# nannau/DoWnGAN

Measured on AMD Instinct MI355X. Metric: train-step samples/sec (G+D+GP), higher is better.
Workload: dtype bf16

## Files before the change

downgan_amd/_lib.py:

```python
from __future__ import annotations

import ctypes as C
import os

_HERE = os.path.dirname(os.path.abspath(__file__))
LIB_PATH = os.environ.get("DG_LIB_OVERRIDE") or os.path.join(_HERE, "csrc", "libdowngan_hip.so")

DG_F32, DG_BF16 = 0, 1
STATUS = {0: "DG_OK", -1: "DG_ERR_BAD_SHAPE", -2: "DG_ERR_BAD_DTYPE", -3: "DG_ERR_BAD_ARG", -4: "DG_ERR_LAUNCH"}


class Epilogue(C.Structure):
    _fields_ = [("bias", C.c_void_p), ("has_act", C.c_int), ("act_slope", C.c_float),
                ("r1", C.c_void_p), ("ldr1", C.c_int64), ("s1", C.c_float),
                ("r2", C.c_void_p), ("ldr2", C.c_int64), ("s2", C.c_float),
                ("mask", C.c_void_p), ("ldmask", C.c_int64), ("mask_slope", C.c_float),
                ("accumulate", C.c_int), ("mask_bits", C.c_void_p), ("out_bits", C.c_void_p),
                ("mask_c0", C.c_int), ("mask_last", C.c_int), ("out_q", C.c_void_p), ("out_qs", C.c_void_p), ("ldqs", C.c_int64),
                ("out_u", C.c_void_p), ("out_ue", C.c_void_p), ("skip_y", C.c_int), ("out_amax", C.c_void_p)]


class ConvGeom(C.Structure):
    _fields_ = [("dtype", C.c_int), ("N", C.c_int), ("H", C.c_int), ("W", C.c_int),
                ("Cin", C.c_int), ("Cout", C.c_int), ("stride", C.c_int), ("cin_real", C.c_int), ("pixel_shuffle", C.c_int),
# ... 48 lines not shown
EOF_MAX_C, EOF_MAX_K = 8, 64
RAPSD_MAX_N = 2048


class EofFields(C.Structure):
    _fields_ = [("base", C.c_void_p), ("dtype", C.c_int), ("T", C.c_int), ("C", C.c_int), ("P", C.c_int),
                ("ld_t", C.c_int64), ("ld_c", C.c_int64), ("ld_p", C.c_int64)]


MINMAX_PARTS = 256
_vp, _i, _i64, _f = C.c_void_p, C.c_int, C.c_int64, C.c_float
_PROTOS = {
    "dg_conv3x3_fwd": [C.POINTER(ConvGeom), C.POINTER(Epilogue), _vp, _vp, _vp, _vp],
    "dg_conv3x3_dgrad": [C.POINTER(ConvGeom), C.POINTER(Epilogue), _vp, _vp, _vp, _vp],
    "dg_conv3x3_wgrad": [C.POINTER(ConvGeom), _vp, _vp, _vp, _vp, _vp],
    "dg_conv3x3_wgrad_dense": [_vp, _i, _vp, _vp, _vp, _vp, _vp],
    "dg_conv3x3_wgrad_f8": [C.POINTER(ConvGeom), _vp, _vp, _vp, _vp, _vp, _vp],
    "dg_exp_from_amax": [_vp, _i, _i, _vp, _vp],
    "dg_conv3x3_wgrad_dense_f8": [C.POINTER(ConvGeom), _i, _vp, _vp, _vp, _vp, _vp, _vp],
    "dg_gather_gemm": [C.POINTER(GGDesc), C.POINTER(Epilogue), _vp, _vp, _vp, _vp],
    "dg_conv3x3_plan": [C.POINTER(ConvGeom), _i, C.POINTER(GGDesc)],
    "dg_last_conv_kernels": [],
    "dg_conv3x3_dgrad_launches": [C.POINTER(ConvGeom)],
    "dg_colsum": [_i, _vp, _i64, _i64, _i64, _i64, _i, _vp, _vp],
    "dg_colsum_multi": [_i, _vp, _i64, _i64, _i, _i, _vp, _vp],
    "dg_repack_conv_weights": [_i, _i, _vp, _vp, _i, _i, _vp],
    "dg_repack_dense_dgrad": [_i, _vp, _i, _i, _vp, _vp],
    "dg_wgrad_unswap": [_vp, _vp, _i, _i, _vp],
    "dg_linear_fwd": [_i, _vp, _i64, _vp, _i64, _vp, _i, _i, _i, _i64, _vp],
    "dg_linear_dx": [_i, _i, _vp, _i, _vp, _i64, _vp, _i64, _vp, _i64, _f, _i, _i, _i64, _vp],
    "dg_linear_dw": [_i, _vp, _i, _vp, _i64, _vp, _i64, _i, _i, _i64, _vp],
    "dg_linear_dw_wide": [_i, _vp, _i, _vp, _i64, _vp, _i64, _i, _i, _i64, _i, _vp],
    "dg_bias_act": [_i, _vp, _i, _vp, _vp, _i, _i, _i, _i, _f, _vp, _i, _f, _vp],
    "dg_mask_mul": [_i, _vp, _i64, _vp, _i64, _i64, _i, _f, _vp],
    "dg_axpby": [_i, _vp, _i64, _vp, _i64, _f, _vp, _i64, _f, _i64, _i, _vp],
    "dg_gp_interp": [_i, _vp, _vp, _vp, _vp, _i, _i64, _vp],
    "dg_gp_interp_c2": [_i, _vp, _vp, _i64, _vp, _vp, _vp, _vp, _i, _i64, _vp],
    "dg_scale_rows_c2": [_i, _vp, _i64, _vp, _vp, _i, _i64, _vp],
    "dg_sumsq_rows": [_i, _vp, _i, _i64, _vp, _vp],
    "dg_gp_finish": [_vp, _i, _i, _f, _f, _vp, _vp, _vp],
    "dg_scale_rows": [_i, _vp, _vp, _vp, _i, _i64, _vp],
    "dg_l1": [_i, _vp, _i64, _vp, _i64, _i64, _i, _vp, _vp, _i64, _f, _vp, _i64, _vp],
    "dg_sqdiff": [_i, _vp, _i64, _vp, _i64, _i64, _i, _vp, _vp],
    "dg_sum_strided": [_vp, _i, _i, _f, _vp, _vp],
    "dg_fill_col": [_vp, _i, _i, _i, _f, _vp],
    "dg_adam": [_vp, _vp, _vp, _vp, _vp, _i64, _f, _f, _f, _f, _i, _f, _vp],
# ... 94 lines not shown
```

downgan_amd/csrc/conv_halo.hip:

```cpp
#include "gg_common.h"

#ifdef DG_STAMP
__device__ unsigned long long g_stamps[2 * 8 * 12];
extern "C" int dg_debug_stamps(unsigned long long* out) {
  return hipMemcpyFromSymbol(out, HIP_SYMBOL(g_stamps), sizeof(g_stamps)) == hipSuccess ? 0 : 1;
}
#define DG_WGLOG_MAX 16384
__device__ unsigned long long g_wglog[DG_WGLOG_MAX * 3];
extern "C" int dg_debug_wglog(unsigned long long* out, int n) {
  return hipMemcpyFromSymbol(out, HIP_SYMBOL(g_wglog), sizeof(unsigned long long) * 3 * (n < DG_WGLOG_MAX ? n : DG_WGLOG_MAX)) == hipSuccess ? 0 : 1;
}
#define STAMP(v) do { __builtin_amdgcn_sched_barrier(0); v = __builtin_amdgcn_s_memtime(); __builtin_amdgcn_sched_barrier(0); } while (0)
#else
#define STAMP(v) do { } while (0)
#endif
bool gg_regroup_taps_by_plane(GGArgs& a) {
  if (a.ntaps != 9) return false;
  unsigned codes[9], out[9];
  bool seen[3][3] = {};
  for (int t = 0; t < 9; ++t) {
    codes[t] = t < 8 ? (unsigned)((a.tap_lo >> (8 * t)) & 0xffull) : (a.tap_hi & 0xffu);
    const int dy = (int)(codes[t] & 3u) - 1, dx = (int)((codes[t] >> 2) & 3u) - 1;
    if (dy < -1 || dy > 1 || dx < -1 || dx > 1 || seen[dy + 1][dx + 1]) return false;
    seen[dy + 1][dx + 1] = true;
  }
  int n = 0;
  for (int plane = 0; plane < 4; ++plane)
    for (int t = 0; t < 9; ++t) {
      const int dy = (int)(codes[t] & 3u) - 1, dx = (int)((codes[t] >> 2) & 3u) - 1;
      if ((dy != 0) * 2 + (dx != 0) != plane) continue;
      const unsigned by = dy == -1 ? 0u : 1u, bx = dx == -1 ? 0u : 1u;
      out[n++] = by | (bx << 2) | (codes[t] & 0xf0u);
    }
  a.tap_lo = 0; a.tap_hi = 0;
  for (int t = 0; t < 9; ++t) {
    if (t < 8) a.tap_lo |= (unsigned long long)out[t] << (8 * t); else a.tap_hi = out[t];
  }
  return true;
}

template <typename T, bool S2, bool PS = false, int NW = 4, bool SEG = false>
__global__ __launch_bounds__(64 * NW, 2) void gg_halo4w_kernel(const GGArgs a, int tiles_x, int tiles_y) {
  static_assert(!SEG || (!S2 && !PS && NW == 4), "SEG is a mode of the plain four-wave kernel");
  constexpr int NT = 64 * NW, RPP = NT / 8;
  constexpr int EPC = DT<T>::EPC;
  constexpr int ES = (int)sizeof(T);
  constexpr int TH = 16, TW = 16, PW = TW + 2, PROWS = (TH + 2) * PW;
  constexpr int BC = 32 * NW, KC = 8;
  constexpr int PITCH = KC * 16 + 16;
  constexpr int WROW = KC * 16;
  constexpr int NPL = (PROWS * KC + NT - 1) / NT;
  constexpr int NWL = BC * KC / NT;
  extern __shared__ __attribute__((aligned(16))) char dsm4w[];
  char* const s_patch = dsm4w;
  char* const s_w = dsm4w + PROWS * PITCH;

  const int tid = threadIdx.x, lane = tid & 63, wave = __builtin_amdgcn_readfirstlane(tid >> 6);
  const unsigned tile = SEG ? blockIdx.x : xcd_remap(blockIdx.x, a.nwg);
  const int tile_c = tile % a.nct;
  unsigned rest = tile / a.nct;
  const int tx0 = (rest % tiles_x) * TW; rest /= tiles_x;
  int cls = 0;
  if (SEG && a.seg == 2) { cls = (int)(rest & 3u); rest >>= 2; }
  const int ty0 = (rest % tiles_y) * TH; rest /= tiles_y;
  if (SEG && a.seg != 2) { cls = (int)(rest & 3u); rest >>= 2; }
  const int img = (int)rest;
  const int ntaps_l = SEG ? (0x4221 >> (4 * cls)) & 15 : a.ntaps;
  const int tap0_l = SEG ? (0x5310 >> (4 * cls)) & 15 : 0;
  const int c0 = tile_c * BC;
  const int cc = tid & 7, r0 = tid >> 3;
  const int wq = wave & 3, wh = wave >> 2;
  const int sy_base = S2 ? (ty0 > 0 ? 2 * (ty0 - 1) : 0) : (ty0 - 1 > 0 ? ty0 - 1 : 0);
  const char* Xb = PS ? reinterpret_cast<const char*>(a.x) + ((long long)img * 2 * a.Hs + 2 * sy_base) * (2 * a.Ws) * a.ldx * ES
                      : reinterpret_cast<const char*>(a.x) + ((long long)img * a.Hs + sy_base) * a.Ws * a.ldx * ES;
  const char* Wb = reinterpret_cast<const char*>(a.w) + (long long)c0 * a.ldw * ES;
  const int l15 = lane & 15, g = lane >> 4;
  const int ncbr = a.cch / KC;
  const int ncb = S2 ? 4 * ncbr : ncbr;
  const int nsteps = ncbr * ntaps_l;
  auto plane_of = [&](int vcb) { return S2 ? (int)(vcb >= ncbr) + (int)(vcb >= 2 * ncbr) + (int)(vcb >= 3 * ncbr) : 0; };
  auto ntaps_of = [&](int vcb) { return S2 ? (0x4221 >> (4 * plane_of(vcb))) & 15 : ntaps_l; };

  unsigned woff[NWL];
#pragma unroll
  for (int i = 0; i < NWL; ++i) {
    int row = wave * 32 + i * 8 + (lane >> 3);
    const int logical = (lane & 7) ^ ((row >> 1) & 7);
    row = perm64(row);
    if (c0 + row >= a.Nout) row = a.Nout - 1 - c0;
    woff[i] = (unsigned)((long long)row * a.ldw * ES) + logical * 16;
  }
  auto tap_code = [&](int vcb, int tap) {
    const int gt = S2 ? ((0x5310 >> (4 * plane_of(vcb))) & 15) + tap : tap0_l + tap;
    return gt < 8 ? (unsigned)((a.tap_lo >> (8 * gt)) & 0xffull) : (a.tap_hi & 0xffu);
  };
  constexpr int K1 = RPP / PW, K2 = RPP % PW;
  const int p_rstep = (S2 ? 2 : PS ? 4 : 1) * a.Ws * a.ldx * ES, p_cstep = ((S2 || PS) ? 2 : 1) * a.ldx * ES;
  const int p_A = K1 * p_rstep + K2 * p_cstep, p_Bd = p_rstep - PW * p_cstep;
  unsigned p_off0, p_wlo = 0, p_whb = 0;
  {
    const int py0 = r0 / PW, px0 = r0 - py0 * PW;
    const int o_rows = S2 ? 2 * (ty0 - 1) - sy_base : PS ? 4 * (ty0 - 1 - sy_base) : ty0 - 1 - sy_base;
    const int o_cols = (S2 || PS) ? 2 * (tx0 - 1) : tx0 - 1;
    p_off0 = (unsigned)((o_rows * a.Ws + o_cols) * a.ldx * ES + py0 * p_rstep + px0 * p_cstep) + cc * 16;
    const unsigned hlim = S2 ? (unsigned)a.Hs >> 1 : (unsigned)a.Hs, wlim = S2 ? (unsigned)a.Ws >> 1 : (unsigned)a.Ws;
#pragma unroll
    for (int i = 0; i < NPL; ++i) {
      const int w = (px0 + i * K2) / PW;
      const int py = py0 + i * K1 + w, px = px0 + i * K2 - w * PW;
      const bool ok = r0 + RPP * i < PROWS && (unsigned)(ty0 - 1 + py) < hlim && (unsigned)(tx0 - 1 + px) < wlim;
      if (i < 8) p_wlo |= (unsigned)w << (4 * i); else p_whb |= (unsigned)w << (4 * (i - 8));
      if (!ok) p_whb |= 1u << (16 + i);
    }
  }
  asm volatile("" : "+v"(p_off0), "+v"(p_wlo), "+v"(p_whb));
  u32x4_t rp[NPL];
  auto load_patch = [&](int vcb) {
    const int plane = plane_of(vcb), cb = vcb - plane * ncbr;
    const int ppy = plane >> 1, ppx = plane & 1;
    const int psq = PS ? (cb * KC) / a.cps_src_chunks : 0;
    const int psy = psq >> 1, psx = psq & 1;
    long long cboff = PS ? (long long)(cb * KC - psq * a.cps_src_chunks) * EPC * ES : (long long)cb * KC * EPC * ES;
    if (S2) cboff += (long long)(ppy * a.Ws + ppx) * a.ldx * ES;
    if (PS) cboff += (long long)(psy * 2 * a.Ws + psx) * a.ldx * ES;
    const unsigned long long xbase = (unsigned long long)(Xb + cboff);
    const unsigned long long xuni = ((unsigned long long)(unsigned)__builtin_amdgcn_readfirstlane((int)(unsigned)(xbase >> 32)) << 32) |
                                    (unsigned)__builtin_amdgcn_readfirstlane((int)(unsigned)xbase);
    __amdgpu_buffer_rsrc_t rx = __builtin_amdgcn_make_buffer_rsrc((void*)xuni, 0, (int)DG_OOB_OFF, 0x00020000);
#pragma unroll
    for (int i = 0; i < NPL; ++i) {
      const int w = (int)__builtin_amdgcn_ubfe(i < 8 ? p_wlo : p_whb, i < 8 ? 4 * i : 4 * (i - 8), 4);
      const unsigned bad = (unsigned)__builtin_amdgcn_sbfe((int)p_whb, 16 + i, 1);
      const unsigned off = ((unsigned)__mul24(w, p_Bd) + p_off0 + (unsigned)(i * p_A)) | bad;
      rp[i] = __builtin_amdgcn_raw_buffer_load_b128(rx, off, 0, 0);
      __builtin_amdgcn_sched_barrier(0);
    }
  };
  char* const st_base = s_patch + r0 * PITCH + cc * 16;
  auto store_patch = [&]() {
#pragma unroll
    for (int i = 0; i < NPL; ++i) {
      const int pr = r0 + RPP * i;
      if (pr < PROWS) *reinterpret_cast<uint4*>(st_base + i * RPP * PITCH) = __builtin_bit_cast(uint4, rp[i]);
    }
  };
  typedef int i32x4h_t __attribute__((ext_vector_type(4)));
  i32x4h_t w_rs;
  int w_dst0 = 0;
  auto dma_setup = [&](int vcb, int tap, int slot) {
    const unsigned code = tap_code(vcb, tap);
    const long long wo = (long long)(code >> 4) * a.Cred + (vcb - plane_of(vcb) * ncbr) * KC * EPC;
    const unsigned long long wbase = (unsigned long long)(Wb + wo * ES);
    w_rs[0] = __builtin_amdgcn_readfirstlane((int)(unsigned)wbase);
    w_rs[1] = __builtin_amdgcn_readfirstlane((int)(unsigned)(wbase >> 32) & 0xffff);
    w_rs[2] = (int)DG_OOB_OFF;
    w_rs[3] = 0x00020000;
    w_dst0 = __builtin_amdgcn_readfirstlane(
        (int)(unsigned long long)((__attribute__((address_space(3))) char*)(s_w + slot * (BC * WROW) + (wave * 32) * WROW)));
  };
  auto dma_piece = [&](int i) {
    asm volatile("s_mov_b32 m0, %0\n\ts_nop 0\n\tbuffer_load_dwordx4 %1, %2, 0 offen lds"
                 :: "s"(w_dst0 + i * 8 * WROW), "v"(woff[i]), "s"(w_rs) : "memory");
  };
  auto dma_w = [&](int cb, int tap, int slot) {
    dma_setup(cb, tap, slot);
#pragma unroll
    for (int i = 0; i < NWL; ++i) dma_piece(i);
  };
  auto barrier_all = [&]() { asm volatile("s_waitcnt vmcnt(0)" ::: "memory"); __syncthreads(); };
  auto barrier_keep_patch = [&]() { asm volatile("s_waitcnt vmcnt(%0)" :: "n"(NPL) : "memory"); __syncthreads(); };

  constexpr bool PREB = sizeof(T) == 2;
  f32x4_t acc[8][4];
#pragma unroll
  for (int j = 0; j < 8; ++j) {
    f32x4_t b = f32x4_t{0.f, 0.f, 0.f, 0.f};
    const int cbq = c0 + (tid >> 8) * 128 + (j >> 2) * 64 + 16 * ((tid & 63) >> 4) + 4 * (j & 3);
    if (PREB && a.bias && cbq < a.Nout) { const float4 b4 = *reinterpret_cast<const float4*>(a.bias + cbq); b = f32x4_t{b4.x, b4.y, b4.z, b4.w}; }
#pragma unroll
    for (int i = 0; i < 4; ++i) acc[j][i] = b;
  }

  const char* fa_k[2];
#pragma unroll
  for (int kk = 0; kk < 2; ++kk) fa_k[kk] = s_w + (wh * 128 + l15) * WROW + (((kk * 4 + g) ^ ((l15 >> 1) & 7)) * 16);
  const char* const fb_lane = s_patch + l15 * PITCH + g * 16;
  auto read_frags = [&](uint4 (&fa)[8], uint4 (&fb)[4], int pa, const char* pb, int kk) {
#pragma unroll
    for (int j = 0; j < 8; ++j) fa[j] = *reinterpret_cast<const uint4*>(fa_k[kk] + pa + j * 16 * WROW);
#pragma unroll
    for (int i = 0; i < 4; ++i) fb[i] = *reinterpret_cast<const uint4*>(pb + i * PW * PITCH + kk * 64);
  };
  auto mma_rows = [&](const uint4 (&fa)[8], const uint4 (&fb)[4], int j0) {
#pragma unroll
    for (int j = j0; j < j0 + 2; ++j)
#pragma unroll
      for (int i = 0; i < 4; ++i) Mma<T>::run(fa[j], fb[i], acc[j][i]);
  };
  auto adv = [&](int& c_, int& t_) { if (++t_ == ntaps_of(c_)) { t_ = 0; ++c_; } };
  auto patch_ptr = [&](int vcb_, int tap_) -> const char* {
    const unsigned code = tap_code(vcb_, tap_);
    const int dy = (int)(code & 3u) - 1, dx = (int)((code >> 2) & 3u) - 1;
    return fb_lane + ((wq * 4 + 1 + dy) * PW + 1 + dx) * PITCH;
  };
// ... 1 lines not shown
#ifdef DG_STAMP
  unsigned long long tK0 = 0, tA = 0, tB = 0, tC = 0, tD = 0, tE = 0, sAB = 0, sBC = 0, sCD = 0, sDE = 0, tL0 = 0;
  STAMP(tK0);
#endif
  load_patch(0);
  int cb = 0, tap = 0, cbw = 0, tapw = 0;
  dma_w(0, 0, 0);
  adv(cbw, tapw);
  if (nsteps > 1) dma_w(cbw, tapw, 1);
  adv(cbw, tapw);
  store_patch();
  barrier_all();
  uint4 fa[8], fb[4];
  const char* pb = patch_ptr(0, 0);
  int pa = 0;
  read_frags(fa, fb, pa, pb, 0);
  STAMP(tL0);
  for (int s = 0; s < nsteps; ++s) {
    STAMP(tA);
    const bool more = s + 1 < nsteps;
    int ntap = tap + 1, ncbn = cb;
    const int ntaps_cb = ntaps_of(cb);
    if (ntap == ntaps_cb) { ntap = 0; ncbn = cb + 1; }
    const bool swap = ntap == 0 && more;
    const bool patch_now = cb + 1 < ncb && (ntaps_cb == 1 || tap == 0);
    const bool fetch = s + 2 < nsteps;
#pragma unroll
    for (int q = 0; q < 4; ++q) {
      mma_rows(fa, fb, 2 * q);
      asm volatile("" : "+v"(acc[2 * q][0]), "+v"(acc[2 * q][1]), "+v"(acc[2 * q][2]), "+v"(acc[2 * q][3]),
                        "+v"(acc[2 * q + 1][0]), "+v"(acc[2 * q + 1][1]), "+v"(acc[2 * q + 1][2]), "+v"(acc[2 * q + 1][3]) :: "memory");
      __builtin_amdgcn_sched_barrier(0);
      fa[2 * q] = *reinterpret_cast<const uint4*>(fa_k[1] + pa + (2 * q) * 16 * WROW);
      fa[2 * q + 1] = *reinterpret_cast<const uint4*>(fa_k[1] + pa + (2 * q + 1) * 16 * WROW);
      asm volatile("" ::: "memory"); __builtin_amdgcn_sched_barrier(0);
    }
#pragma unroll
    for (int i = 0; i < 4; ++i) fb[i] = *reinterpret_cast<const uint4*>(pb + i * PW * PITCH + 64);
    __builtin_amdgcn_sched_barrier(0);
    if (patch_now) load_patch(cb + 1);
    __builtin_amdgcn_sched_barrier(0);
    STAMP(tB);
#pragma unroll
    for (int q = 0; q < 4; ++q) mma_rows(fa, fb, 2 * q);
    __builtin_amdgcn_sched_barrier(0);
    STAMP(tC);
    if (patch_now && !swap) barrier_keep_patch(); else barrier_all();
    STAMP(tD);
    pa = ((s + 1) & 1) * (BC * WROW);
    pb = patch_ptr(ncbn < ncb ? ncbn : 0, ntap);
    if (swap) {
      store_patch();
      barrier_all();
    }
    if (more) read_frags(fa, fb, pa, pb, 0);
    __builtin_amdgcn_sched_barrier(0);
    if (fetch) { dma_setup(cbw, tapw, s & 1);
#pragma unroll
      for (int q = 0; q < 4; ++q) dma_piece(q);
    }
    adv(cbw, tapw);
    __builtin_amdgcn_sched_barrier(0);
    tap = ntap; cb = ncbn;
    STAMP(tE);
#ifdef DG_STAMP
    sAB += tB - tA; sBC += tC - tB; sCD += tD - tC; sDE += tE - tD;
#endif
  }
#ifdef DG_STAMP
  unsigned long long tL1, tX;
  STAMP(tL1);
#endif
#ifdef DG_STAMP
  unsigned long long est[4] = {0, 0, 0, 0};
  halo_epilogue<T, 2, PREB>(a, acc, img, ty0, tx0, c0 + wh * 128, wq, 0, l15, g, SEG ? cls >> 1 : -1, SEG ? cls & 1 : -1, est);
#else
  if constexpr (SEG) halo_epilogue<T, 2, PREB>(a, acc, img, ty0, tx0, c0 + wh * 128, wq, 0, l15, g, cls >> 1, cls & 1);
  else halo_epilogue<T, 2, PREB>(a, acc, img, ty0, tx0, c0 + wh * 128, wq, 0, l15, g);
#endif
#ifdef DG_STAMP
  STAMP(tX);
  if (blockIdx.x < DG_WGLOG_MAX && tid == 0) {
    unsigned hw, xcc;
    asm volatile("s_getreg_b32 %0, hwreg(HW_REG_HW_ID)" : "=s"(hw));
    asm volatile("s_getreg_b32 %0, hwreg(HW_REG_XCC_ID)" : "=s"(xcc));
    unsigned long long* o = g_wglog + (unsigned long long)blockIdx.x * 3;
    o[0] = (unsigned long long)hw | ((unsigned long long)xcc << 32); o[1] = tK0; o[2] = tX;
  }
  const unsigned sb = blockIdx.x - a.nwg / 2;
  if (sb < 2u && lane == 0) {
    unsigned long long* o = g_stamps + (sb * 8 + wave) * 12;
    o[0] = sAB; o[1] = sBC; o[2] = sCD; o[3] = sDE; o[4] = (unsigned long long)nsteps; o[5] = tL1 - tL0; o[6] = tX - tL1; o[7] = tL0 - tK0;
    o[8] = est[0] - tL1; o[9] = est[1] - est[0]; o[10] = est[2] - est[1]; o[11] = est[3] - est[2];
  }
#endif
}

template <typename T, bool S2, bool PS = false, int NW = 4, bool SEG = false>
static int gg_launch_halo4w(GGArgs& a, int N, hipStream_t st) {
  constexpr int BC = 32 * NW;
  constexpr int LDS_BYTES = 324 * 144 + 2 * BC * 128;
  DG_SET_MAX_LDS_ONCE((&gg_halo4w_kernel<T, S2, PS, NW, SEG>), LDS_BYTES);
  const int tiles_x = (a.Wg + 15) / 16, tiles_y = (a.Hg + 15) / 16;
  a.nct = (unsigned)((a.Nout + BC - 1) / BC);
  a.nwg = a.nct * (unsigned)(tiles_x * tiles_y * N) * (SEG ? 4u : 1u);
  g_last_kinds |= 8;
#ifdef DG_STAMP
  static const int abl = getenv("DG_ABL") ? atoi(getenv("DG_ABL")) : 0;
  a.dbg = abl;
  if (abl & 2) {
    hipFuncSetAttribute((const void*)&gg_halo4w_kernel<T, S2, PS, NW, SEG>, hipFuncAttributeMaxDynamicSharedMemorySize, 100 * 1024);
    hipLaunchKernelGGL((gg_halo4w_kernel<T, S2, PS, NW, SEG>), dim3(a.nwg), dim3(64 * NW), 100 * 1024, st, a, tiles_x, tiles_y);
    return dg_check_launch();
  }
#endif
  hipLaunchKernelGGL((gg_halo4w_kernel<T, S2, PS, NW, SEG>), dim3(a.nwg), dim3(64 * NW), LDS_BYTES, st, a, tiles_x, tiles_y);
  return dg_check_launch();
}

int gg_launch_halo(GGArgs& a, int dtype, int N, bool s2, bool ps, int nw, hipStream_t st) {
  if (!gg_halo_row_step_ok(a.Ws, a.ldx, dtype, ps ? 4 : s2 ? 2 : 1)) return DG_ERR_BAD_SHAPE;
  if (a.seg) return dtype == DG_BF16 ? gg_launch_halo4w<bf16_t, false, false, 4, true>(a, N, st) : gg_launch_halo4w<float, false, false, 4, true>(a, N, st);
  if (dtype == DG_F32) {
    if (ps) return gg_launch_halo4w<float, false, true>(a, N, st);
    return s2 ? gg_launch_halo4w<float, true>(a, N, st) : gg_launch_halo4w<float, false>(a, N, st);
  }
  if (ps) return gg_launch_halo4w<bf16_t, false, true>(a, N, st);
  if (s2) return nw == 8 ? gg_launch_halo4w<bf16_t, true, false, 8>(a, N, st) : gg_launch_halo4w<bf16_t, true>(a, N, st);
  return gg_launch_halo4w<bf16_t, false>(a, N, st);
}
```

downgan_amd/csrc/conv_plan.hip:

```cpp
#include "gg_common.h"

thread_local int g_last_kinds = 0;

static int gg_validate(const dg_gg_desc* d, bool f8 = false, bool compact_src = false) {
  if (d->dtype != DG_F32 && d->dtype != DG_BF16) return DG_ERR_BAD_DTYPE;
  const int epc = f8 ? 16 : d->dtype == DG_F32 ? 4 : 8;
  if (d->N <= 0 || d->Hs <= 0 || d->Ws <= 0 || d->Hg <= 0 || d->Wg <= 0 || d->Hd <= 0 || d->Wd <= 0) return DG_ERR_BAD_SHAPE;
  if (d->Cred <= 0 || d->Cred % 8 || d->Nout <= 0 || d->Nout % 16) return DG_ERR_BAD_SHAPE;
  if (d->ntaps < 1 || d->ntaps > 9) return DG_ERR_BAD_SHAPE;
  if ((compact_src ? d->lds % 2 || d->lds < 2 : d->lds % epc) || d->ldd % 4 || d->ldw % epc) return DG_ERR_BAD_SHAPE;
  for (int t = 0; t < d->ntaps; ++t) {
    if (d->tap_dy[t] < -1 || d->tap_dy[t] > 1 || d->tap_dx[t] < -1 || d->tap_dx[t] > 1) return DG_ERR_BAD_ARG;
    if (d->tap_w[t] < 0 || d->tap_w[t] > 8) return DG_ERR_BAD_ARG;
  }
  if (d->src_ps && ((d->Cred / 4) % 8)) return DG_ERR_BAD_SHAPE;
  if (d->dst_ps && ((d->Nout / 4) % 16)) return DG_ERR_BAD_SHAPE;
  if ((long long)d->N * d->Hg * d->Wg >= (1ll << 31)) return DG_ERR_BAD_SHAPE;
  if (d->dst_ps) {
    if (2 * d->Hg > d->Hd || 2 * d->Wg > d->Wd) return DG_ERR_BAD_SHAPE;
  } else {
    if ((d->Hg - 1) * d->dy_mul + d->dy_off >= d->Hd || (d->Wg - 1) * d->dx_mul + d->dx_off >= d->Wd) return DG_ERR_BAD_SHAPE;
    if (d->dy_off < 0 || d->dx_off < 0 || d->dy_mul < 1 || d->dx_mul < 1) return DG_ERR_BAD_SHAPE;
  }
  return DG_OK;
// ... 20 lines not shown
    GGArgs b = a;
    if (gg_regroup_taps_by_plane(b)) {
      return gg_launch_halo(b, dtype, N, true, false, (dtype == DG_BF16 && b.Nout % 256 == 0) ? 8 : 4, st);
    }
  }
  if (a.Nout <= 16 && a.sy_mul == 1 && a.sx_mul == 1 && !a.src_ps && !a.dst_ps && a.cch % 8 == 0 && a.Hg >= 8 &&
      a.Wg >= 8 && a.ntaps >= 2 && a.Hs == a.Hg && a.Ws == a.Wg && !a.mask_bits && !a.out_bits)
    return gg_launch_halo16(a, dtype, N, st);
  return gg_launch_rows(a, dtype, st);
}

static int gg_launch_f8(GGArgs& a, const F8Args& f, int N, hipStream_t st) {
  if (a.cch % 8 || a.Nout <= 64 || a.Hg < 8 || a.Wg < 8 || a.src_ps) return DG_ERR_BAD_SHAPE;
  if (a.sy_mul == 1 && a.sx_mul == 1 && a.Hs == a.Hg && a.Ws == a.Wg) return gg_launch_halo_f8(a, f, N, false, 4, st);
  if (a.sy_mul == 2 && a.sx_mul == 2 && a.Hs == 2 * a.Hg && a.Ws == 2 * a.Wg && a.dy_mul == 1 && a.dx_mul == 1 && !a.dst_ps) {
    GGArgs b = a;
    if (gg_regroup_taps_by_plane(b)) {
      return gg_launch_halo_f8(b, f, N, true, b.Nout % 256 == 0 ? 8 : 4, st);
    }
  }
  return DG_ERR_BAD_SHAPE;
}
static int gather_gemm_impl(const dg_gg_desc* d, const dg_epilogue* ep, const void* x, const void* w, void* y, void* stream,
                            bool im2col_small, const dg_f8_operands* f8 = nullptr, bool seg = false) {
  if (!d || !x || !w || !y) return DG_ERR_BAD_ARG;
  if (f8 && (d->dtype != DG_BF16 || !f8->xs || !f8->ws || d->Cred % 128)) return DG_ERR_BAD_SHAPE;
  int rc = gg_validate(d, f8 != nullptr, im2col_small);
  if (rc) return rc;
  const int epc = f8 ? 16 : d->dtype == DG_F32 ? 4 : 8;
  GGArgs a{};
  a.x = x; a.w = w; a.y = y;
  a.ldx = d->lds; a.ldw = d->ldw; a.ldy = d->ldd;
  a.M = d->N * d->Hg * d->Wg; a.Hg = d->Hg; a.Wg = d->Wg; a.Hs = d->Hs; a.Ws = d->Ws;
  a.Cred = d->Cred; a.cch = d->Cred / epc; a.ntaps = d->ntaps; a.kchunks = d->ntaps * a.cch;
  a.sy_mul = d->sy_mul; a.sx_mul = d->sx_mul;
  a.tap_lo = 0; a.tap_hi = 0;
  for (int t = 0; t < d->ntaps; ++t) {
    unsigned long long code = (unsigned)(d->tap_dy[t] + 1) | ((unsigned)(d->tap_dx[t] + 1) << 2) | ((unsigned)d->tap_w[t] << 4);
    if (t < 8) a.tap_lo |= code << (8 * t); else a.tap_hi = (unsigned)code;
  }
  a.Nout = d->Nout; a.Hd = d->Hd; a.Wd = d->Wd;
  a.dy_mul = d->dy_mul; a.dx_mul = d->dx_mul; a.dy_off = d->dy_off; a.dx_off = d->dx_off;
  a.src_ps = d->src_ps; a.dst_ps = d->dst_ps;
  a.cps_src_chunks = d->src_ps ? d->Cred / 4 / epc : 1;
  a.cps_dst = d->dst_ps ? d->Nout / 4 : d->Nout;
  a.s1 = a.s2 = 1.f; a.mask_slope = 1.f; a.act_slope = 1.f;
  if (ep) {
// ... 11 lines not shown
    a.no_y = ep->skip_y ? 1 : 0;
    if (a.no_y && ((!a.out_q && !a.out_u) || a.accumulate)) return DG_ERR_BAD_ARG;
    a.out_amax = (unsigned*)ep->out_amax;
    if (((a.out_u && !a.out_q) || a.out_amax) && !im2col_small) return DG_ERR_BAD_SHAPE;
    if (a.out_u && (d->dtype != DG_BF16 || d->Nout < 128 || d->Nout % 64 || d->dst_ps)) return DG_ERR_BAD_SHAPE;
    if ((a.out_q != nullptr) != (a.out_qs != nullptr)) return DG_ERR_BAD_ARG;
    if (a.out_q && (d->dtype != DG_BF16 || d->Nout < 128 || d->Nout % 64)) return DG_ERR_BAD_SHAPE;
    const int cdst = d->dst_ps ? d->Nout / 4 : d->Nout;
    if (a.out_q && d->dst_ps && (cdst % 32 || a.out_u || a.mask_bits || a.out_bits)) return DG_ERR_BAD_SHAPE;
    a.ldqs = ep->ldqs > 0 ? (int)ep->ldqs : cdst / 32;
    a.qs_shift = 0;
    if (a.out_q && (a.ldqs != cdst / 32 || d->dst_ps)) {
      const int n16 = cdst / 16;
      if ((n16 & (n16 - 1)) || a.ldqs < cdst / 32) return DG_ERR_BAD_SHAPE;
      while ((1 << a.qs_shift) < n16) ++a.qs_shift;
    }
    if ((a.mask_bits || a.out_bits) && (d->Nout < 128 || d->Nout % 64 || d->dst_ps || (a.mask_bits && a.mask))) return DG_ERR_BAD_SHAPE;
    if ((a.r1 && a.ldr1 % 4) || (a.r2 && a.ldr2 % 4) || (a.mask && a.ldmask % 4)) return DG_ERR_BAD_SHAPE;
  }
  hipStream_t st = reinterpret_cast<hipStream_t>(stream);
  a.seg = seg ? 1 : 0;
  if (seg) {
    if ((long long)d->Cred * d->Nout * 18 <= (2ll << 20)) a.seg = 2;
  }
  if (f8) {
    F8Args f{(const unsigned char*)f8->xs, (const unsigned char*)f8->ws, f8->ldxs > 0 ? (int)f8->ldxs : f8->ldxs < 0 ? 0 : d->Cred / 32};
    if (f8->ldxs >= 0 && (f.ldxs < d->Cred / 32 || f.ldxs % 4)) return DG_ERR_BAD_SHAPE;
    return gg_launch_f8(a, f, d->N, st);
  }
  static const bool no_im2col = getenv("DG_GG_NOIM2COL") != nullptr;
  if (im2col_small && !no_im2col) return gg_launch_im2col(a, d->dtype, st);
  return gg_launch(a, d->dtype, d->N, st);
}

extern "C" int dg_gather_gemm(const dg_gg_desc* d, const dg_epilogue* ep, const void* x, const void* w,
                              void* y, void* stream) {
  return gather_gemm_impl(d, ep, x, w, y, stream, false);
}

static int geom_validate(const dg_conv_geom* g) {
  if (!g) return DG_ERR_BAD_ARG;
  if (g->dtype != DG_F32 && g->dtype != DG_BF16) return DG_ERR_BAD_DTYPE;
  if (g->N <= 0 || g->H <= 0 || g->W <= 0) return DG_ERR_BAD_SHAPE;
  if (g->stride != 1 && g->stride != 2) return DG_ERR_BAD_SHAPE;
  if (g->stride == 2 && ((g->H | g->W) & 1)) return DG_ERR_BAD_SHAPE;
  if (g->Cin <= 0 || g->Cin % 8 || g->Cout <= 0 || g->Cout % 16) return DG_ERR_BAD_SHAPE;
// ... 60 lines not shown
  const int epc = d[0].dtype == DG_F32 ? 4 : 8;
  if (n != 4 || d[0].src_ps || d[0].dst_ps || (d[0].Cred / epc) % 8 || d[0].Nout <= 64 || d[0].Hg < 8 || d[0].Wg < 8) return false;
  if (d[0].ntaps != 1 || d[1].ntaps != 2 || d[2].ntaps != 2 || d[3].ntaps != 4) return false;
  if (!gg_halo_row_step_ok(d[0].Ws, d[0].lds, d[0].dtype, 1)) return false;
  *out = d[3];
  out->ntaps = 0;
  for (int c = 0; c < 4; ++c) {
    if (d[c].dy_off != (c >> 1) || d[c].dx_off != (c & 1) || d[c].dy_mul != 2 || d[c].dx_mul != 2) return false;
    for (int t = 0; t < d[c].ntaps; ++t, ++out->ntaps) {
      out->tap_dy[out->ntaps] = d[c].tap_dy[t]; out->tap_dx[out->ntaps] = d[c].tap_dx[t]; out->tap_w[out->ntaps] = d[c].tap_w[t];
    }
  }
  return out->ntaps == 9;
}

extern "C" int dg_conv3x3_dgrad(const dg_conv_geom* g, const dg_epilogue* ep, const void* dy, const void* w_dgrad,
                                void* dx, void* stream) {
  if (g && g->Cin % 16) return DG_ERR_BAD_SHAPE;
  dg_gg_desc d[4];
  g_last_kinds = 0;
  int n = dg_conv3x3_plan(g, 1, d);
  if (n < 0) return n;
  dg_gg_desc ds;
  if (seg_dgrad_desc(d, n, &ds)) return gather_gemm_impl(&ds, ep, dy, w_dgrad, dx, stream, false, nullptr, true);
  for (int i = 0; i < n; ++i) {
    int rc = dg_gather_gemm(&d[i], ep, dy, w_dgrad, dx, stream);
    if (rc) return rc;
  }
  return DG_OK;
}

extern "C" int dg_conv3x3_fwd_f8(const dg_conv_geom* g, const dg_epilogue* ep, const dg_f8_operands* q, void* y, void* stream) {
  if (!q || !g || g->dtype != DG_BF16 || g->Cin % 128) return DG_ERR_BAD_SHAPE;
  dg_gg_desc d[4];
  g_last_kinds = 0;
  int n = dg_conv3x3_plan(g, 0, d);
  if (n < 0) return n;
  d[0].lds = q->ldxq;
  return gather_gemm_impl(&d[0], ep, q->xq, q->wq, y, stream, false, q);
}

extern "C" int dg_conv3x3_dgrad_f8(const dg_conv_geom* g, const dg_epilogue* ep, const dg_f8_operands* q, void* dx, void* stream) {
  if (!q || !g || g->dtype != DG_BF16 || g->pixel_shuffle || g->Cout % 128 || g->Cin % 16) return DG_ERR_BAD_SHAPE;
  dg_gg_desc d[4];
  g_last_kinds = 0;
  int n = dg_conv3x3_plan(g, 1, d);
  if (n < 0) return n;
  dg_gg_desc ds;
  if (seg_dgrad_desc(d, n, &ds) && ds.Cred % 128 == 0) {
    ds.lds = q->ldxq;
    return gather_gemm_impl(&ds, ep, q->xq, q->wq, dx, stream, false, q, true);
  }
  for (int i = 0; i < n; ++i) {
    d[i].lds = q->ldxq;
    int rc = gather_gemm_impl(&d[i], ep, q->xq, q->wq, dx, stream, false, q);
    if (rc) return rc;
  }
  return DG_OK;
}

extern "C" int dg_last_conv_kernels(void) { return g_last_kinds; }

extern "C" int dg_conv3x3_dgrad_launches(const dg_conv_geom* g) {
  dg_gg_desc d[4], ds;
  const int n = dg_conv3x3_plan(g, 1, d);
  if (n < 0) return n;
  return seg_dgrad_desc(d, n, &ds) ? 1 : n;
}
```

downgan_amd/csrc/gg_common.h:

```cpp
#pragma once
#include "dg_internal.h"

#include <stdlib.h>
#include <type_traits>


extern thread_local int g_last_kinds;

struct GGArgs {
  const void* x; const void* w; void* y;
  const float* bias; const void* r1; const void* r2; const void* mask;
  const void* mask_bits; void* out_bits;
  void* out_q; void* out_qs;
  void* out_u; const unsigned char* out_ue;
  int no_y;
  unsigned* out_amax;
  int ldqs, qs_shift;
  long long ldx, ldw, ldy, ldr1, ldr2, ldmask;
  int M, Hg, Wg, Hs, Ws;
  int cch, kchunks, Cred, ntaps;
  int sy_mul, sx_mul;
  unsigned long long tap_lo; unsigned tap_hi;
  int Nout, Hd, Wd, dy_mul, dx_mul, dy_off, dx_off;
  int src_ps, dst_ps, cps_src_chunks, cps_dst;
  int has_act, accumulate;
  float act_slope, s1, s2, mask_slope;
  unsigned nwg, nct;
  int mask_c0, mask_last;
  int seg;
  int dbg;
};

typedef __attribute__((ext_vector_type(4))) unsigned int u32x4_t;
#define DG_OOB_OFF 0x80000000u

__host__ __device__ constexpr int perm64(int r) { return (r & ~63) | ((r & 0x0c) << 2) | ((r >> 2) & 0x0c) | (r & 3); }

typedef __attribute__((ext_vector_type(2))) unsigned int u32x2_t;
template <typename T> struct EpiV;
template <> struct EpiV<bf16_t> {
  static constexpr int CPU = 8, NU = 2;
  static __device__ __forceinline__ void unpack(const u32x4_t& t, float* v) {
#pragma unroll
    for (int q = 0; q < 4; ++q) { v[2 * q] = __uint_as_float(t[q] << 16); v[2 * q + 1] = __uint_as_float(t[q] & 0xffff0000u); }
  }
  static __device__ __forceinline__ u32x4_t pack(const float* v) {
    u32x4_t t;
#pragma unroll
    for (int q = 0; q < 4; ++q) t[q] = pack_bf16x2(v[2 * q], v[2 * q + 1]);
    return t;
  }
};
template <> struct EpiV<float> {
  static constexpr int CPU = 4, NU = 4;
// ... 483 lines not shown
```

include/downgan_hip.h:

```cpp
#ifndef DOWNGAN_HIP_H
#define DOWNGAN_HIP_H

#include <stddef.h>
#include <stdint.h>

#ifdef __cplusplus
extern "C" {
#endif

#define DG_F32 0
#define DG_BF16 1

typedef enum dg_status {
  DG_OK = 0,
  DG_ERR_BAD_SHAPE = -1,
  DG_ERR_BAD_DTYPE = -2,
  DG_ERR_BAD_ARG = -3,
  DG_ERR_LAUNCH = -4
} dg_status;

typedef struct dg_epilogue {
  const float* bias;
  int has_act;
  float act_slope;
// ... 51 lines not shown

int dg_conv3x3_wgrad_dense(const dg_conv_geom* g, int nconv, const void* x, const void* dy,
                           float* const* dw, float* const* db, void* stream);

int dg_conv3x3_wgrad_f8(const dg_conv_geom* g, const void* xq, const void* ex, const void* dyq, const void* ey, float* dw,
                        void* stream);

int dg_conv3x3_wgrad_dense_f8(const dg_conv_geom* g, int nconv, const void* xq, const void* ex, const void* dyq, const void* ey,
                              float* const* dw, void* stream);

int dg_colsum(int dtype, const void* dy, int64_t rows_outer, int64_t ld_outer, int64_t rows_inner,
              int64_t ld, int C, float* db, void* stream);

int dg_colsum_multi(int dtype, const void* dy, int64_t rows, int64_t ld, int C, int nseg, float* const* db, void* stream);

int dg_gather_gemm(const dg_gg_desc* d, const dg_epilogue* ep, const void* x, const void* w, void* y,
                   void* stream);

int dg_last_conv_kernels(void);

int dg_conv3x3_plan(const dg_conv_geom* g, int kind, dg_gg_desc* out);

int dg_conv3x3_dgrad_launches(const dg_conv_geom* g);

int dg_repack_conv_weights(int dtype, int kind, const float* master, void* dst, int CoutP, int CinP,
                           void* stream);
int dg_repack_dense_dgrad(int dtype, const float* const* masters, int nconv, int F, void* dst, void* stream);
int dg_wgrad_unswap(const float* tmp, float* dw, int CoutP, int CinP, void* stream);


int dg_linear_fwd(int dtype, const void* x, int64_t ldx, const void* w, int64_t ldw, float* y,
                  int ldy, int B, int O, int64_t K, void* stream);
int dg_linear_dx(int dtype, int out_dtype, const float* dy, int ldo, const void* w, int64_t ldw,
                 void* dx, int64_t lddx, const void* mask, int64_t ldmask, float mask_slope, int B,
                 int O, int64_t K, void* stream);
int dg_linear_dw(int dtype, const float* dy, int ldo, const void* x, int64_t ldx, float* dw,
                 int64_t lddw, int B, int O, int64_t K, void* stream);
int dg_linear_dw_wide(int dtype, const float* dy, int ldo, const void* x, int64_t ldx, float* dw,
                      int64_t lddw, int B, int O, int64_t K, int accumulate, void* stream);


int dg_bias_act(int out_dtype, const float* in, int ldi, const float* bias, void* out, int ldo,
                int rows, int C, int has_act, float slope, const void* mask, int ldmask,
                float mask_slope, void* stream);
int dg_mask_mul(int dtype, void* u, int64_t ldu, const void* y, int64_t ldy, int64_t rows, int C,
                float slope, void* stream);
// ... 142 lines not shown
```

Before: 71.06.

## Walk all four dgrad parity classes in one workgroup for small-channel bf16 convs

Adds a WALK mode to the segmented stride-2 dgrad halo kernel. For bf16 with at most 16 channel chunks, each workgroup now processes all four output parity classes in sequence instead of launching four times as many workgroups. Channel blocks are walked in serpentine order so the staged input patch is reused across class boundaries, and an epilogue plus accumulator reset runs at each class end. This cuts redundant patch loads and workgroup count at the cost of a longer serial chain per workgroup and less parallelism; a per-class entry point keeps the old path for comparison.

```diff
diff --git a/downgan_amd/_lib.py b/downgan_amd/_lib.py
--- a/downgan_amd/_lib.py
+++ b/downgan_amd/_lib.py
@@ -94,6 +94,7 @@
     "dg_conv3x3_plan": [C.POINTER(ConvGeom), _i, C.POINTER(GGDesc)],
     "dg_last_conv_kernels": [],
     "dg_conv3x3_dgrad_launches": [C.POINTER(ConvGeom)],
+    "dg_conv3x3_dgrad_per_class": [C.POINTER(ConvGeom), C.POINTER(Epilogue), _vp, _vp, _vp, _vp],
     "dg_colsum": [_i, _vp, _i64, _i64, _i64, _i64, _i, _vp, _vp],
     "dg_colsum_multi": [_i, _vp, _i64, _i64, _i, _i, _vp, _vp],
     "dg_repack_conv_weights": [_i, _i, _vp, _vp, _i, _i, _vp],
diff --git a/downgan_amd/csrc/conv_halo.hip b/downgan_amd/csrc/conv_halo.hip
--- a/downgan_amd/csrc/conv_halo.hip
+++ b/downgan_amd/csrc/conv_halo.hip
@@ -39,9 +39,10 @@
   return true;
 }
 
-template <typename T, bool S2, bool PS = false, int NW = 4, bool SEG = false>
+template <typename T, bool S2, bool PS = false, int NW = 4, bool SEG = false, bool WALK = false>
 __global__ __launch_bounds__(64 * NW, 2) void gg_halo4w_kernel(const GGArgs a, int tiles_x, int tiles_y) {
   static_assert(!SEG || (!S2 && !PS && NW == 4), "SEG is a mode of the plain four-wave kernel");
+  static_assert(!WALK || SEG, "WALK is a form of the SEG launch");
   constexpr int NT = 64 * NW, RPP = NT / 8;
   constexpr int EPC = DT<T>::EPC;
   constexpr int ES = (int)sizeof(T);
@@ -61,9 +62,9 @@
   unsigned rest = tile / a.nct;
   const int tx0 = (rest % tiles_x) * TW; rest /= tiles_x;
   int cls = 0;
-  if (SEG && a.seg == 2) { cls = (int)(rest & 3u); rest >>= 2; }
+  if (SEG && !WALK && a.seg == 2) { cls = (int)(rest & 3u); rest >>= 2; }
   const int ty0 = (rest % tiles_y) * TH; rest /= tiles_y;
-  if (SEG && a.seg != 2) { cls = (int)(rest & 3u); rest >>= 2; }
+  if (SEG && !WALK && a.seg != 2) { cls = (int)(rest & 3u); rest >>= 2; }
   const int img = (int)rest;
   const int ntaps_l = SEG ? (0x4221 >> (4 * cls)) & 15 : a.ntaps;
   const int tap0_l = SEG ? (0x5310 >> (4 * cls)) & 15 : 0;
@@ -76,10 +77,15 @@
   const char* Wb = reinterpret_cast<const char*>(a.w) + (long long)c0 * a.ldw * ES;
   const int l15 = lane & 15, g = lane >> 4;
   const int ncbr = a.cch / KC;
-  const int ncb = S2 ? 4 * ncbr : ncbr;
-  const int nsteps = ncbr * ntaps_l;
-  auto plane_of = [&](int vcb) { return S2 ? (int)(vcb >= ncbr) + (int)(vcb >= 2 * ncbr) + (int)(vcb >= 3 * ncbr) : 0; };
-  auto ntaps_of = [&](int vcb) { return S2 ? (0x4221 >> (4 * plane_of(vcb))) & 15 : ntaps_l; };
+  const int ncb = (S2 || WALK) ? 4 * ncbr : ncbr;
+  const int nsteps = WALK ? 9 * ncbr : ncbr * ntaps_l;
+  auto plane_of = [&](int vcb) { return (S2 || WALK) ? (int)(vcb >= ncbr) + (int)(vcb >= 2 * ncbr) + (int)(vcb >= 3 * ncbr) : 0; };
+  auto cls_of = [&](int vcb) { return (0x0213 >> (4 * plane_of(vcb))) & 15; };
+  auto cbr_of = [&](int vcb) {
+    const int k = plane_of(vcb);
+    return WALK && (k & 1) ? (k + 1) * ncbr - 1 - vcb : vcb - k * ncbr;
+  };
+  auto ntaps_of = [&](int vcb) { return S2 ? (0x4221 >> (4 * plane_of(vcb))) & 15 : WALK ? (0x4221 >> (4 * cls_of(vcb))) & 15 : ntaps_l; };
 
   unsigned woff[NWL];
 #pragma unroll
@@ -91,7 +97,7 @@
     woff[i] = (unsigned)((long long)row * a.ldw * ES) + logical * 16;
   }
   auto tap_code = [&](int vcb, int tap) {
-    const int gt = S2 ? ((0x5310 >> (4 * plane_of(vcb))) & 15) + tap : tap0_l + tap;
+    const int gt = S2 ? ((0x5310 >> (4 * plane_of(vcb))) & 15) + tap : WALK ? ((0x5310 >> (4 * cls_of(vcb))) & 15) + tap : tap0_l + tap;
     return gt < 8 ? (unsigned)((a.tap_lo >> (8 * gt)) & 0xffull) : (a.tap_hi & 0xffu);
   };
   constexpr int K1 = RPP / PW, K2 = RPP % PW;
@@ -116,7 +122,7 @@
   asm volatile("" : "+v"(p_off0), "+v"(p_wlo), "+v"(p_whb));
   u32x4_t rp[NPL];
   auto load_patch = [&](int vcb) {
-    const int plane = plane_of(vcb), cb = vcb - plane * ncbr;
+    const int plane = S2 ? plane_of(vcb) : 0, cb = cbr_of(vcb);
     const int ppy = plane >> 1, ppx = plane & 1;
     const int psq = PS ? (cb * KC) / a.cps_src_chunks : 0;
     const int psy = psq >> 1, psx = psq & 1;
@@ -127,6 +133,7 @@
     const unsigned long long xuni = ((unsigned long long)(unsigned)__builtin_amdgcn_readfirstlane((int)(unsigned)(xbase >> 32)) << 32) |
                                     (unsigned)__builtin_amdgcn_readfirstlane((int)(unsigned)xbase);
     __amdgpu_buffer_rsrc_t rx = __builtin_amdgcn_make_buffer_rsrc((void*)xuni, 0, (int)DG_OOB_OFF, 0x00020000);
+    if constexpr (WALK) asm volatile("" : "+v"(p_off0), "+v"(p_wlo), "+v"(p_whb));
 #pragma unroll
     for (int i = 0; i < NPL; ++i) {
       const int w = (int)__builtin_amdgcn_ubfe(i < 8 ? p_wlo : p_whb, i < 8 ? 4 * i : 4 * (i - 8), 4);
@@ -149,7 +156,7 @@
   int w_dst0 = 0;
   auto dma_setup = [&](int vcb, int tap, int slot) {
     const unsigned code = tap_code(vcb, tap);
-    const long long wo = (long long)(code >> 4) * a.Cred + (vcb - plane_of(vcb) * ncbr) * KC * EPC;
+    const long long wo = (long long)(code >> 4) * a.Cred + cbr_of(vcb) * KC * EPC;
     const unsigned long long wbase = (unsigned long long)(Wb + wo * ES);
     w_rs[0] = __builtin_amdgcn_readfirstlane((int)(unsigned)wbase);
     w_rs[1] = __builtin_amdgcn_readfirstlane((int)(unsigned)(wbase >> 32) & 0xffff);
@@ -172,14 +179,17 @@
 
   constexpr bool PREB = sizeof(T) == 2;
   f32x4_t acc[8][4];
-#pragma unroll
-  for (int j = 0; j < 8; ++j) {
-    f32x4_t b = f32x4_t{0.f, 0.f, 0.f, 0.f};
-    const int cbq = c0 + (tid >> 8) * 128 + (j >> 2) * 64 + 16 * ((tid & 63) >> 4) + 4 * (j & 3);
-    if (PREB && a.bias && cbq < a.Nout) { const float4 b4 = *reinterpret_cast<const float4*>(a.bias + cbq); b = f32x4_t{b4.x, b4.y, b4.z, b4.w}; }
-#pragma unroll
-    for (int i = 0; i < 4; ++i) acc[j][i] = b;
-  }
+  auto init_acc = [&](const GGArgs& aa, int tid_) {
+#pragma unroll
+    for (int j = 0; j < 8; ++j) {
+      f32x4_t b = f32x4_t{0.f, 0.f, 0.f, 0.f};
+      const int cbq = c0 + (tid_ >> 8) * 128 + (j >> 2) * 64 + 16 * ((tid_ & 63) >> 4) + 4 * (j & 3);
+      if (PREB && aa.bias && cbq < aa.Nout) { const float4 b4 = *reinterpret_cast<const float4*>(aa.bias + cbq); b = f32x4_t{b4.x, b4.y, b4.z, b4.w}; }
+#pragma unroll
+      for (int i = 0; i < 4; ++i) acc[j][i] = b;
+    }
+  };
+  init_acc(a, tid);
 
   const char* fa_k[2];
 #pragma unroll
@@ -227,8 +237,10 @@
     int ntap = tap + 1, ncbn = cb;
     const int ntaps_cb = ntaps_of(cb);
     if (ntap == ntaps_cb) { ntap = 0; ncbn = cb + 1; }
-    const bool swap = ntap == 0 && more;
-    const bool patch_now = cb + 1 < ncb && (ntaps_cb == 1 || tap == 0);
+    const bool newpatch = cb + 1 < ncb && (!WALK || cbr_of(cb + 1) != cbr_of(cb));
+    const bool patch_now = newpatch && (ntaps_cb == 1 || tap == 0);
+    const bool swap = ntap == 0 && newpatch;
+    const bool cls_end = WALK && ntap == 0 && (!more || plane_of(cb + 1) != plane_of(cb));
     const bool fetch = s + 2 < nsteps;
 #pragma unroll
     for (int q = 0; q < 4; ++q) {
@@ -258,6 +270,27 @@
       store_patch();
       barrier_all();
     }
+    if (cls_end) {
+      if (fetch) { dma_setup(cbw, tapw, s & 1);
+#pragma unroll
+        for (int q = 0; q < 4; ++q) dma_piece(q);
+      }
+      adv(cbw, tapw);
+      __builtin_amdgcn_sched_barrier(0);
+      typedef const __attribute__((address_space(4))) GGArgs GGArgsK;
+      GGArgsK* ak = (GGArgsK*)__builtin_amdgcn_kernarg_segment_ptr();
+      asm volatile("" : "+s"(ak));
+      const GGArgs& ae = *(const GGArgs*)ak;
+      int tid_e = tid;
+      asm volatile("" : "+v"(tid_e));
+      const int ecls = cls_of(cb);
+      halo_epilogue<T, 2, PREB>(ae, acc, img, ty0, tx0, c0 + wh * 128, wq, 0, tid_e & 15, (tid_e & 63) >> 4, ecls >> 1, ecls & 1);
+#pragma unroll
+      for (int i = 0; i < NPL; ++i) asm volatile("" : "=v"(rp[i]));
+      init_acc(ae, tid_e);
+      read_frags(fa, fb, pa, pb, 0);
+      __builtin_amdgcn_sched_barrier(0);
+    } else {
     if (more) read_frags(fa, fb, pa, pb, 0);
     __builtin_amdgcn_sched_barrier(0);
     if (fetch) { dma_setup(cbw, tapw, s & 1);
@@ -266,6 +299,7 @@
     }
     adv(cbw, tapw);
     __builtin_amdgcn_sched_barrier(0);
+    }
     tap = ntap; cb = ncbn;
     STAMP(tE);
 #ifdef DG_STAMP
@@ -278,9 +312,10 @@
 #endif
 #ifdef DG_STAMP
   unsigned long long est[4] = {0, 0, 0, 0};
-  halo_epilogue<T, 2, PREB>(a, acc, img, ty0, tx0, c0 + wh * 128, wq, 0, l15, g, SEG ? cls >> 1 : -1, SEG ? cls & 1 : -1, est);
+  if constexpr (!WALK) halo_epilogue<T, 2, PREB>(a, acc, img, ty0, tx0, c0 + wh * 128, wq, 0, l15, g, SEG ? cls >> 1 : -1, SEG ? cls & 1 : -1, est);
 #else
-  if constexpr (SEG) halo_epilogue<T, 2, PREB>(a, acc, img, ty0, tx0, c0 + wh * 128, wq, 0, l15, g, cls >> 1, cls & 1);
+  if constexpr (WALK) { }
+  else if constexpr (SEG) halo_epilogue<T, 2, PREB>(a, acc, img, ty0, tx0, c0 + wh * 128, wq, 0, l15, g, cls >> 1, cls & 1);
   else halo_epilogue<T, 2, PREB>(a, acc, img, ty0, tx0, c0 + wh * 128, wq, 0, l15, g);
 #endif
 #ifdef DG_STAMP
@@ -301,31 +336,36 @@
 #endif
 }
 
-template <typename T, bool S2, bool PS = false, int NW = 4, bool SEG = false>
+template <typename T, bool S2, bool PS = false, int NW = 4, bool SEG = false, bool WALK = false>
 static int gg_launch_halo4w(GGArgs& a, int N, hipStream_t st) {
   constexpr int BC = 32 * NW;
   constexpr int LDS_BYTES = 324 * 144 + 2 * BC * 128;
-  DG_SET_MAX_LDS_ONCE((&gg_halo4w_kernel<T, S2, PS, NW, SEG>), LDS_BYTES);
+  DG_SET_MAX_LDS_ONCE((&gg_halo4w_kernel<T, S2, PS, NW, SEG, WALK>), LDS_BYTES);
   const int tiles_x = (a.Wg + 15) / 16, tiles_y = (a.Hg + 15) / 16;
   a.nct = (unsigned)((a.Nout + BC - 1) / BC);
-  a.nwg = a.nct * (unsigned)(tiles_x * tiles_y * N) * (SEG ? 4u : 1u);
+  a.nwg = a.nct * (unsigned)(tiles_x * tiles_y * N) * (SEG && !WALK ? 4u : 1u);
   g_last_kinds |= 8;
 #ifdef DG_STAMP
   static const int abl = getenv("DG_ABL") ? atoi(getenv("DG_ABL")) : 0;
   a.dbg = abl;
   if (abl & 2) {
-    hipFuncSetAttribute((const void*)&gg_halo4w_kernel<T, S2, PS, NW, SEG>, hipFuncAttributeMaxDynamicSharedMemorySize, 100 * 1024);
-    hipLaunchKernelGGL((gg_halo4w_kernel<T, S2, PS, NW, SEG>), dim3(a.nwg), dim3(64 * NW), 100 * 1024, st, a, tiles_x, tiles_y);
+    hipFuncSetAttribute((const void*)&gg_halo4w_kernel<T, S2, PS, NW, SEG, WALK>, hipFuncAttributeMaxDynamicSharedMemorySize, 100 * 1024);
+    hipLaunchKernelGGL((gg_halo4w_kernel<T, S2, PS, NW, SEG, WALK>), dim3(a.nwg), dim3(64 * NW), 100 * 1024, st, a, tiles_x, tiles_y);
     return dg_check_launch();
   }
 #endif
-  hipLaunchKernelGGL((gg_halo4w_kernel<T, S2, PS, NW, SEG>), dim3(a.nwg), dim3(64 * NW), LDS_BYTES, st, a, tiles_x, tiles_y);
+  hipLaunchKernelGGL((gg_halo4w_kernel<T, S2, PS, NW, SEG, WALK>), dim3(a.nwg), dim3(64 * NW), LDS_BYTES, st, a, tiles_x, tiles_y);
   return dg_check_launch();
 }
 
 int gg_launch_halo(GGArgs& a, int dtype, int N, bool s2, bool ps, int nw, hipStream_t st) {
   if (!gg_halo_row_step_ok(a.Ws, a.ldx, dtype, ps ? 4 : s2 ? 2 : 1)) return DG_ERR_BAD_SHAPE;
-  if (a.seg) return dtype == DG_BF16 ? gg_launch_halo4w<bf16_t, false, false, 4, true>(a, N, st) : gg_launch_halo4w<float, false, false, 4, true>(a, N, st);
+  if (a.seg) {
+    const bool per_class = dtype != DG_BF16 || (a.seg & DG_SEG_PER_CLASS) || a.cch > 16;
+    a.seg &= ~DG_SEG_PER_CLASS;
+    if (!per_class) return gg_launch_halo4w<bf16_t, false, false, 4, true, true>(a, N, st);
+    return dtype == DG_BF16 ? gg_launch_halo4w<bf16_t, false, false, 4, true>(a, N, st) : gg_launch_halo4w<float, false, false, 4, true>(a, N, st);
+  }
   if (dtype == DG_F32) {
     if (ps) return gg_launch_halo4w<float, false, true>(a, N, st);
     return s2 ? gg_launch_halo4w<float, true>(a, N, st) : gg_launch_halo4w<float, false>(a, N, st);
diff --git a/downgan_amd/csrc/conv_plan.hip b/downgan_amd/csrc/conv_plan.hip
--- a/downgan_amd/csrc/conv_plan.hip
+++ b/downgan_amd/csrc/conv_plan.hip
@@ -66,7 +66,7 @@
   return DG_ERR_BAD_SHAPE;
 }
 static int gather_gemm_impl(const dg_gg_desc* d, const dg_epilogue* ep, const void* x, const void* w, void* y, void* stream,
-                            bool im2col_small, const dg_f8_operands* f8 = nullptr, bool seg = false) {
+                            bool im2col_small, const dg_f8_operands* f8 = nullptr, int seg = 0) {
   if (!d || !x || !w || !y) return DG_ERR_BAD_ARG;
   if (f8 && (d->dtype != DG_BF16 || !f8->xs || !f8->ws || d->Cred % 128)) return DG_ERR_BAD_SHAPE;
   int rc = gg_validate(d, f8 != nullptr, im2col_small);
@@ -124,6 +124,7 @@
   a.seg = seg ? 1 : 0;
   if (seg) {
     if ((long long)d->Cred * d->Nout * 18 <= (2ll << 20)) a.seg = 2;
+    if (seg == 2) a.seg |= DG_SEG_PER_CLASS;
   }
   if (f8) {
     F8Args f{(const unsigned char*)f8->xs, (const unsigned char*)f8->ws, f8->ldxs > 0 ? (int)f8->ldxs : f8->ldxs < 0 ? 0 : d->Cred / 32};
@@ -230,7 +231,7 @@
   int n = dg_conv3x3_plan(g, 1, d);
   if (n < 0) return n;
   dg_gg_desc ds;
-  if (seg_dgrad_desc(d, n, &ds)) return gather_gemm_impl(&ds, ep, dy, w_dgrad, dx, stream, false, nullptr, true);
+  if (seg_dgrad_desc(d, n, &ds)) return gather_gemm_impl(&ds, ep, dy, w_dgrad, dx, stream, false, nullptr, 1);
   for (int i = 0; i < n; ++i) {
     int rc = dg_gather_gemm(&d[i], ep, dy, w_dgrad, dx, stream);
     if (rc) return rc;
@@ -238,6 +239,18 @@
   return DG_OK;
 }
 
+extern "C" int dg_conv3x3_dgrad_per_class(const dg_conv_geom* g, const dg_epilogue* ep, const void* dy, const void* w_dgrad,
+                                          void* dx, void* stream) {
+  if (g && g->Cin % 16) return DG_ERR_BAD_SHAPE;
+  dg_gg_desc d[4];
+  g_last_kinds = 0;
+  int n = dg_conv3x3_plan(g, 1, d);
+  if (n < 0) return n;
+  dg_gg_desc ds;
+  if (!seg_dgrad_desc(d, n, &ds)) return DG_ERR_BAD_SHAPE;
+  return gather_gemm_impl(&ds, ep, dy, w_dgrad, dx, stream, false, nullptr, 2);
+}
+
 extern "C" int dg_conv3x3_fwd_f8(const dg_conv_geom* g, const dg_epilogue* ep, const dg_f8_operands* q, void* y, void* stream) {
   if (!q || !g || g->dtype != DG_BF16 || g->Cin % 128) return DG_ERR_BAD_SHAPE;
   dg_gg_desc d[4];
@@ -257,7 +270,7 @@
   dg_gg_desc ds;
   if (seg_dgrad_desc(d, n, &ds) && ds.Cred % 128 == 0) {
     ds.lds = q->ldxq;
-    return gather_gemm_impl(&ds, ep, q->xq, q->wq, dx, stream, false, q, true);
+    return gather_gemm_impl(&ds, ep, q->xq, q->wq, dx, stream, false, q, 1);
   }
   for (int i = 0; i < n; ++i) {
     d[i].lds = q->ldxq;
diff --git a/downgan_amd/csrc/gg_common.h b/downgan_amd/csrc/gg_common.h
--- a/downgan_amd/csrc/gg_common.h
+++ b/downgan_amd/csrc/gg_common.h
@@ -30,6 +30,8 @@
   int seg;
   int dbg;
 };
+
+#define DG_SEG_PER_CLASS 4
 
 typedef __attribute__((ext_vector_type(4))) unsigned int u32x4_t;
 #define DG_OOB_OFF 0x80000000u
diff --git a/include/downgan_hip.h b/include/downgan_hip.h
--- a/include/downgan_hip.h
+++ b/include/downgan_hip.h
@@ -97,6 +97,9 @@
 int dg_conv3x3_plan(const dg_conv_geom* g, int kind, dg_gg_desc* out);
 
 int dg_conv3x3_dgrad_launches(const dg_conv_geom* g);
+
+int dg_conv3x3_dgrad_per_class(const dg_conv_geom* g, const dg_epilogue* ep, const void* dy,
+                               const void* w_dgrad, void* dx, void* stream);
 
 int dg_repack_conv_weights(int dtype, int kind, const float* master, void* dst, int CoutP, int CinP,
                            void* stream);
```

Result: no change. 71.04, median of 5 (-0.0%).
